# linzhiqiu/t2v_metrics

Hardware: NVIDIA B200
Metric: VQAScore (image,text) pairs/sec @ clip-flant5-xxl, 512px (higher is better)
Workload: dtype bf16

## Files before the change

t2v_metrics_b200/csrc/attention_sm100.cuh:

```cuda
#pragma once
#include "ptx.cuh"
#include "gemm_sm100.cuh"

namespace vqa {

template <typename Kernel, typename... Args>
inline cudaError_t launch_pdl(Kernel kernel, dim3 grid, dim3 block, size_t smem, cudaStream_t stream, Args... args) {
    cudaLaunchConfig_t cfg = {};
    cfg.gridDim = grid;
    cfg.blockDim = block;
    cfg.dynamicSmemBytes = smem;
    cfg.stream = stream;
    cudaLaunchAttribute attrs[1];
    attrs[0].id = cudaLaunchAttributeProgrammaticStreamSerialization;
    attrs[0].val.programmaticStreamSerializationAllowed = 1;
    cfg.attrs = attrs;
    cfg.numAttrs = pdl_enabled() ? 1 : 0;
    return cudaLaunchKernelEx(&cfg, kernel, args...);
}


constexpr int AT_BQ = 128, AT_BK = 128, AT_D = 64;
constexpr int AT_TILE_BYTES = 128 * 64 * 2;
constexpr int AT_TMEM_COLS = 256;
// ... 326 lines not shown
#pragma unroll
            for (int i = 1; i < 6; ++i) bmax_near = fmaxf(bmax_near, sRed[i]);
        }
        const uint64_t cc = pack2(p.scale_log2e, p.scale_log2e);
        const uint32_t bl2 = pack_bf16x2(b_left, b_left), br2 = pack_bf16x2(b_right, b_right);
        auto chunk_max = [](const uint32_t (&v)[32], float& m0, float& m1, float& m2, float& m3) {
#pragma unroll
            for (int i = 0; i < 32; i += 8) {
                m0 = fmax3(m0, __uint_as_float(v[i]), __uint_as_float(v[i + 1]));
                m1 = fmax3(m1, __uint_as_float(v[i + 2]), __uint_as_float(v[i + 3]));
                m2 = fmax3(m2, __uint_as_float(v[i + 4]), __uint_as_float(v[i + 5]));
                m3 = fmax3(m3, __uint_as_float(v[i + 6]), __uint_as_float(v[i + 7]));
            }
        };
        int g = 0;
        for (int qi = 0; qi < nq; ++qi) {
            const int q0 = qi * AT_BQ;
            const int qrow = q0 + row;
            __nv_bfloat16* orow = p.o + (row_base + qrow) * p.ldo + h * AT_D;
            if (q0 + (int)quad * 32 >= len) {
                for (int j = 0; j < nkt; ++j, ++g) {
                    mbar_wait(s_full, (uint32_t)g & 1u);
                    __syncwarp();
                    if (lane == 0) mbar_arrive(s_empty);
                    if (g > 0) mbar_wait(p_full, (uint32_t)(g - 1) & 1u);
                    __syncwarp();
                    if (lane == 0) mbar_arrive(p_full);
                }
                mbar_wait(o_done, (uint32_t)(g - 1) & 1u);
                __syncwarp();
                if (lane == 0) mbar_arrive(o_free);
                if (qrow < p.S) {
#pragma unroll
                    for (int c = 0; c < 8; ++c) *reinterpret_cast<uint4*>(orow + c * 8) = make_uint4(0, 0, 0, 0);
                }
                continue;
            }
            float m_run = 0.f, l_run = 0.f, corr_pend = 1.f;
            bool pend = false;
            for (int j = 0; j < nkt; ++j, ++g) {
                const int k0 = j * AT_BK;
                const int nch = min(4, (len - k0 + 31) >> 5);
                const int dt = j - qi;
                const bool near = HAS_BIAS && (dt <= p.near_tiles) && (dt >= -p.near_tiles);
                const float bias_ub = near ? bmax_near : (dt < 0 ? b_left : b_right);
                const uint32_t s_addr = tmem_S + lane_off;
                mbar_wait(s_full, (uint32_t)g & 1u);
                tcgen05_fence_after();
                if (j == 0) {
                    float a0 = -INFINITY, a1 = -INFINITY, a2 = -INFINITY, a3 = -INFINITY;
#pragma unroll 1
                    for (int c = 0; c < nch; ++c) {
                        uint32_t v[32];
                        tmem_ld_32x32b_x32(s_addr + c * 32, v);
                        tmem_ld_wait();
                        if (k0 + c * 32 + 32 > len) {
#pragma unroll
                            for (int i = 0; i < 32; ++i)
                                if (k0 + c * 32 + i >= len) v[i] = 0xff800000u;
                        }
                        chunk_max(v, a0, a1, a2, a3);
                    }
                    const float raw = fmaxf(fmaxf(a0, a1), fmaxf(a2, a3));
                    m_run = ROUND ? (raw + bias_ub) * p.scale_log2e : fmaf(raw, p.scale_log2e, bias_ub);
                } else {
                    mbar_wait(o_done, (uint32_t)(g - 1) & 1u);
                    tcgen05_fence_after();
                    if (pend) {
#pragma unroll 1
                        for (int c = 0; c < 4; ++c) {
                            uint32_t ov[16];
                            tmem_ld_32x32b_x16(tmem_O + lane_off + c * 16, ov);
                            tmem_ld_wait();
#pragma unroll
                            for (int i = 0; i < 16; ++i) ov[i] = __float_as_uint(__uint_as_float(ov[i]) * corr_pend);
                            tmem_st_32x32b_x16(tmem_O + lane_off + c * 16, ov);
                        }
                        l_run *= corr_pend;
                        pend = false;
                    }
                }
                const float a_add = near ? -m_run : (ROUND ? -m_run : bias_ub - m_run);
                const uint64_t addc = pack2(a_add, a_add);
                const uint32_t bq = near ? smem_u32(sBiasQ) + (uint32_t)(dt * 128 - row + Wn) * BQ_ENTRY : 0u;
                const uint32_t bfar = dt < 0 ? bl2 : br2;
                uint64_t acc0 = 0ull, acc1 = 0ull;
                float t0 = -INFINITY, t1 = -INFINITY, t2 = -INFINITY, t3 = -INFINITY;
                uint32_t bufA[32], bufB[32];
                auto process = [&](uint32_t (&v)[32], int c) {
                    if (c == nch - 1) {
                        tcgen05_fence_before();
                        __syncwarp();
                        if (lane == 0) mbar_arrive(s_empty);
                    }
                    if (k0 + c * 32 + 32 > len) {
#pragma unroll
                        for (int i = 0; i < 32; ++i)
                            if (k0 + c * 32 + i >= len) v[i] = 0xff800000u;
                    }
                    chunk_max(v, t0, t1, t2, t3);
                    uint32_t pk[16];
                    if (near) softmax_chunk<true, POLY, ROUND>(v, pk, bq + c * 32 * BQ_ENTRY, cc, addc, 0u, false, acc0, acc1);
                    else      softmax_chunk<false, POLY, ROUND>(v, pk, 0u, cc, addc, bfar, HAS_BIAS, acc0, acc1);
                    tmem_st_32x32b_x16(tmem_P + lane_off + c * 16, pk);
                };
                tmem_ld_32x32b_x32(s_addr, bufA);
#pragma unroll 1
                for (int c = 0; c < nch; c += 2) {
                    tmem_ld_wait();
                    if (c + 1 < nch) tmem_ld_32x32b_x32(s_addr + (c + 1) * 32, bufB);
                    process(bufA, c);
                    if (c + 1 < nch) {
                        tmem_ld_wait();
                        if (c + 2 < nch) tmem_ld_32x32b_x32(s_addr + (c + 2) * 32, bufA);
                        process(bufB, c + 1);
                    }
                }
                if (nch < 4) {
                    uint32_t z[16];
#pragma unroll
                    for (int i = 0; i < 16; ++i) z[i] = 0u;
#pragma unroll 1
                    for (int c = nch; c < 4; ++c) tmem_st_32x32b_x16(tmem_P + lane_off + c * 16, z);
                }
                {
                    float a0, a1, a2, a3;
                    unpack2(acc0, a0, a1);
                    unpack2(acc1, a2, a3);
                    l_run += (a0 + a1) + (a2 + a3);
                }
                tmem_st_wait();
                tcgen05_fence_before();
                __syncwarp();
                if (lane == 0) mbar_arrive(p_full);
                const float raw = fmaxf(fmaxf(t0, t1), fmaxf(t2, t3));
                const float bound = ROUND ? (raw + bias_ub) * p.scale_log2e : fmaf(raw, p.scale_log2e, bias_ub);
                if (__any_sync(0xffffffffu, bound > m_run + 8.f)) {
                    const float m_new = fmaxf(m_run, bound);
                    corr_pend = fast_exp2(m_run - m_new);
                    m_run = m_new;
                    pend = true;
                }
            }
            mbar_wait(o_done, (uint32_t)(g - 1) & 1u);
            tcgen05_fence_after();
            const float inv = (qrow < len) ? 1.f / l_run : 0.f;
#pragma unroll
            for (int c = 0; c < 2; ++c) {
                uint32_t ov[32];
                tmem_ld_32x32b_x32(tmem_O + lane_off + c * 32, ov);
                tmem_ld_wait();
                if (c == 1) {
                    tcgen05_fence_before();
                    __syncwarp();
                    if (lane == 0) mbar_arrive(o_free);
                }
                if (qrow < p.S) {
#pragma unroll
                    for (int gq = 0; gq < 4; ++gq) {
                        uint32_t w[4];
#pragma unroll
                        for (int e = 0; e < 4; ++e)
                            w[e] = pack_bf16x2(__uint_as_float(ov[gq * 8 + 2 * e]) * inv, __uint_as_float(ov[gq * 8 + 2 * e + 1]) * inv);
                        *reinterpret_cast<uint4*>(orow + c * 32 + gq * 8) = make_uint4(w[0], w[1], w[2], w[3]);
                    }
                }
            }
        }
        tcgen05_fence_before();
    }

    __syncthreads();
    tcgen05_fence_after();
    if (warp == 1) tmem_dealloc<1>(tmem_base, AT_TMEM_COLS);
}

template <bool HAS_BIAS, bool ROUND>
__global__ void __launch_bounds__(320, 2)
attn_tc_d64_split_kernel(const __grid_constant__ CUtensorMap tmap_qkv, const AttnTc2Params p) {
    pdl_launch_dependents();
    pdl_wait();
    constexpr int POLY = 0;
    const int h = blockIdx.y, b = blockIdx.z;
    const int len = p.seq_lens ? min(p.seq_lens[b], p.S) : p.S;
    const uint32_t warp = threadIdx.x >> 5, lane = threadIdx.x & 31u;
    const size_t row_base = (size_t)b * p.S;
    const int nq_all = (len + AT_BQ - 1) / AT_BQ;
    const int nkt = (len + AT_BK - 1) / AT_BK;
    const int q_first = blockIdx.x * p.q_per_cta;
    const int nq = max(0, min(p.q_per_cta, nq_all - q_first));

    if (blockIdx.x == 0) {
        for (int i = threadIdx.x; i < (p.S - nq_all * AT_BQ) * 8; i += blockDim.x) {
            const int r = nq_all * AT_BQ + (i >> 3), c = i & 7;
            *reinterpret_cast<uint4*>(p.o + (row_base + r) * p.ldo + h * AT_D + c * 8) = make_uint4(0, 0, 0, 0);
        }
    }
    if (nq == 0) return;

    extern __shared__ uint8_t at_smem_raw[];
    uint8_t* smem = reinterpret_cast<uint8_t*>((reinterpret_cast<uintptr_t>(at_smem_raw) + 1023) & ~uintptr_t(1023));
    uint8_t* sQ = smem;
    uint8_t* sK = smem + 2 * AT_TILE_BYTES;
    uint8_t* sV = smem + 4 * AT_TILE_BYTES;
    uint8_t* sBiasQ = smem + 6 * AT_TILE_BYTES;
    constexpr uint32_t BQ_ENTRY = ROUND ? 8u : 16u;
    const int Wn = 128 * p.near_tiles + 127;
    const int nQ = HAS_BIAS ? 2 * Wn + 1 : 0;
    float* sRed = reinterpret_cast<float*>(smem + 6 * AT_TILE_BYTES + (((size_t)nQ * BQ_ENTRY + 15) & ~size_t(15)));
    float* sXch = sRed + 16;
    uint64_t* bars = reinterpret_cast<uint64_t*>(sXch + 512);
    uint64_t* q_full = bars;
    uint64_t* q_empty = bars + 2;
    uint64_t* kv_full = bars + 4;
    uint64_t* kv_empty = bars + 6;
    uint64_t* s_full = bars + 8;
    uint64_t* s_empty = bars + 9;
    uint64_t* p_full = bars + 10;
    uint64_t* o_done = bars + 11;
    uint64_t* o_free = bars + 12;
    uint64_t* xbar = bars + 13;
    uint32_t* tmem_ptr_smem = reinterpret_cast<uint32_t*>(bars + 29);

    if (warp == 0 && lane == 0) {
        tma_prefetch_desc(&tmap_qkv);
#pragma unroll
        for (int i = 0; i < 2; ++i) {
            mbar_init(&q_full[i], 1); mbar_init(&q_empty[i], 1);
            mbar_init(&kv_full[i], 1); mbar_init(&kv_empty[i], 1);
        }
        mbar_init(s_full, 1);
        mbar_init(s_empty, 8);
        mbar_init(p_full, 8);
        mbar_init(o_done, 1);
        mbar_init(o_free, 8);
#pragma unroll
        for (int i = 0; i < 16; ++i) mbar_init(&xbar[i], 1);
        fence_barrier_init();
        mbar_arrive_expect_tx(&q_full[0], AT_TILE_BYTES);
        tma_load_2d(sQ, &tmap_qkv, &q_full[0], p.q_col0 + h * AT_D, (int)(row_base + q_first * AT_BQ));
        mbar_arrive_expect_tx(&kv_full[0], 2 * AT_TILE_BYTES);
        tma_load_2d(sK, &tmap_qkv, &kv_full[0], p.k_col0 + h * AT_D, (int)row_base);
        tma_load_2d(sV, &tmap_qkv, &kv_full[0], p.v_col0 + h * AT_D, (int)row_base);
    }
    if (warp == 1) {
        tmem_alloc<1>(tmem_ptr_smem, AT_TMEM_COLS);
        tmem_relinquish<1>();
    }
    const float LOG2E = 1.4426950408889634f;
    const float BSC = ROUND ? 1.0f : LOG2E;
    float b_left = 0.f, b_right = 0.f;
    if (HAS_BIAS) {
        const int width = 2 * p.S - 1;
        const float* src = p.bias_table + (size_t)h * width;
        b_left = __ldg(src) * BSC;
        b_right = __ldg(src + width - 1) * BSC;
        float lmax = -INFINITY;
        for (int x = threadIdx.x; x < nQ; x += blockDim.x) {
            float v[4];
#pragma unroll
            for (int k = 0; k < 4; ++k) {
                const int idx = min(max(x + k - Wn + (p.S - 1), 0), width - 1);
                v[k] = __ldg(src + idx) * BSC;
            }
            if constexpr (ROUND) reinterpret_cast<uint2*>(sBiasQ)[x] = make_uint2(pack_bf16x2(v[0], v[1]), pack_bf16x2(v[2], v[3]));
            else                 reinterpret_cast<float4*>(sBiasQ)[x] = make_float4(v[0], v[1], v[2], v[3]);
            lmax = fmaxf(lmax, v[0]);
        }
#pragma unroll
        for (int o = 16; o > 0; o >>= 1) lmax = fmaxf(lmax, __shfl_xor_sync(0xffffffffu, lmax, o));
        if (lane == 0) sRed[warp] = lmax;
    }
    tcgen05_fence_before();
    __syncthreads();
    tcgen05_fence_after();
    const uint32_t tmem_base = *tmem_ptr_smem;
    const uint32_t tmem_S = tmem_base, tmem_O = tmem_base + 128, tmem_P = tmem_base + 192;
    const int total_tiles = nq * nkt;

    if (warp == 0) {
        if (lane == 0) {
            for (int qi = 0; qi < nq; ++qi) {
                const int qb = qi & 1;
                if (qi > 0) {
                    mbar_wait(&q_empty[qb], (((uint32_t)qi >> 1) & 1u) ^ 1u);
                    mbar_arrive_expect_tx(&q_full[qb], AT_TILE_BYTES);
                    tma_load_2d(sQ + qb * AT_TILE_BYTES, &tmap_qkv, &q_full[qb], p.q_col0 + h * AT_D, (int)(row_base + (q_first + qi) * AT_BQ));
                }
                for (int j = 0; j < nkt; ++j) {
                    const int g = qi * nkt + j;
                    if (g == 0) continue;
                    const int st = g & 1;
                    mbar_wait(&kv_empty[st], (((uint32_t)g >> 1) & 1u) ^ 1u);
                    mbar_arrive_expect_tx(&kv_full[st], 2 * AT_TILE_BYTES);
                    tma_load_2d(sK + st * AT_TILE_BYTES, &tmap_qkv, &kv_full[st], p.k_col0 + h * AT_D, (int)(row_base + j * AT_BK));
                    tma_load_2d(sV + st * AT_TILE_BYTES, &tmap_qkv, &kv_full[st], p.v_col0 + h * AT_D, (int)(row_base + j * AT_BK));
                }
            }
        }
    } else if (warp == 1) {
        if (lane == 0) {
            constexpr uint32_t idesc_s = make_idesc_bf16_f32(128, 128);
            constexpr uint32_t idesc_o = make_idesc_bf16_f32(128, 64) | (1u << 16);
            auto issue_pv = [&](int g) {
                const int j = g % nkt, qi = g / nkt;
                mbar_wait(p_full, (uint32_t)g & 1u);
                if (j == 0 && qi > 0) mbar_wait(o_free, (uint32_t)(qi - 1) & 1u);
                tcgen05_fence_after();
                const uint64_t vdesc = make_mnmajor_sw128_desc(smem_u32(sV + (g & 1) * AT_TILE_BYTES), AT_TILE_BYTES);
#pragma unroll
                for (int ks = 0; ks < AT_BK / 16; ++ks)
                    umma_f16_ts(tmem_O, tmem_P + ks * 8, vdesc + (uint64_t)(ks * (16 * 128 / 16)), idesc_o,
                                (j > 0 || ks > 0) ? 1u : 0u);
                umma_commit<1>(&kv_empty[g & 1]);
                umma_commit<1>(o_done);
            };
            for (int qi = 0; qi < nq; ++qi) {
                const int qb = qi & 1;
                mbar_wait(&q_full[qb], ((uint32_t)qi >> 1) & 1u);
                const uint64_t qdesc = make_kmajor_sw128_desc(smem_u32(sQ + qb * AT_TILE_BYTES));
                for (int j = 0; j < nkt; ++j) {
                    const int g = qi * nkt + j;
                    const int st = g & 1;
                    mbar_wait(&kv_full[st], ((uint32_t)g >> 1) & 1u);
                    mbar_wait(s_empty, ((uint32_t)g & 1u) ^ 1u);
                    tcgen05_fence_after();
                    const uint64_t kdesc = make_kmajor_sw128_desc(smem_u32(sK + st * AT_TILE_BYTES));
#pragma unroll
                    for (int k = 0; k < AT_D / 16; ++k)
                        umma_f16<1>(tmem_S, qdesc + 2 * k, kdesc + 2 * k, idesc_s, k > 0 ? 1u : 0u);
                    umma_commit<1>(s_full);
                    if (j == nkt - 1) umma_commit<1>(&q_empty[qb]);
                    if (g > 0) issue_pv(g - 1);
                }
            }
            issue_pv(total_tiles - 1);
        }
    } else {
        const uint32_t quad = warp & 3u;
        const uint32_t half = (warp - 2u) >> 2;
        const int row = quad * 32 + lane;
        const uint32_t lane_off = (quad * 32u) << 16;
        uint32_t xk = 0;
        auto post = [&](float v) {
            sXch[(xk & 1u) * 256 + half * 128 + row] = v;
            __syncwarp();
            if (lane == 0) mbar_arrive(&xbar[(quad * 2 + half) * 2 + (xk & 1u)]);
        };
        auto collect = [&]() -> float {
            mbar_wait(&xbar[(quad * 2 + (half ^ 1u)) * 2 + (xk & 1u)], (xk >> 1) & 1u);
            const float other = sXch[(xk & 1u) * 256 + (half ^ 1u) * 128 + row];
            ++xk;
            return other;
        };
        float bmax_near = 0.f;
        if (HAS_BIAS) {
            bmax_near = sRed[0];
#pragma unroll
            for (int i = 1; i < 10; ++i) bmax_near = fmaxf(bmax_near, sRed[i]);
        }
        const uint64_t cc = pack2(p.scale_log2e, p.scale_log2e);
        const uint32_t bl2 = pack_bf16x2(b_left, b_left), br2 = pack_bf16x2(b_right, b_right);
        auto chunk_max = [](const uint32_t (&v)[32], float& m0, float& m1, float& m2, float& m3) {
#pragma unroll
            for (int i = 0; i < 32; i += 8) {
                m0 = fmax3(m0, __uint_as_float(v[i]), __uint_as_float(v[i + 1]));
                m1 = fmax3(m1, __uint_as_float(v[i + 2]), __uint_as_float(v[i + 3]));
                m2 = fmax3(m2, __uint_as_float(v[i + 4]), __uint_as_float(v[i + 5]));
                m3 = fmax3(m3, __uint_as_float(v[i + 6]), __uint_as_float(v[i + 7]));
            }
        };
        int g = 0;
        for (int qi = 0; qi < nq; ++qi) {
            const int q0 = (q_first + qi) * AT_BQ;
            const int qrow = q0 + row;
            __nv_bfloat16* orow = p.o + (row_base + qrow) * p.ldo + h * AT_D + half * 32;
            if (q0 + (int)quad * 32 >= len) {
                for (int j = 0; j < nkt; ++j, ++g) {
                    mbar_wait(s_full, (uint32_t)g & 1u);
                    __syncwarp();
                    if (lane == 0) mbar_arrive(s_empty);
                    if (g > 0) mbar_wait(p_full, (uint32_t)(g - 1) & 1u);
                    __syncwarp();
                    if (lane == 0) mbar_arrive(p_full);
                }
                mbar_wait(o_done, (uint32_t)(g - 1) & 1u);
                __syncwarp();
                if (lane == 0) mbar_arrive(o_free);
                if (qrow < p.S) {
#pragma unroll
                    for (int c = 0; c < 4; ++c) *reinterpret_cast<uint4*>(orow + c * 8) = make_uint4(0, 0, 0, 0);
                }
                continue;
            }
            float m_run = 0.f, l_run = 0.f;
            float bound_prev = 0.f;
            for (int j = 0; j < nkt; ++j, ++g) {
                const int k0 = j * AT_BK;
                const int nch = min(4, (len - k0 + 31) >> 5);
                const int c_lo = 2 * (int)half;
                const int n_mine = max(0, min(nch - c_lo, 2));
                const int dt = j - (q_first + qi);
                const bool near = HAS_BIAS && (dt <= p.near_tiles) && (dt >= -p.near_tiles);
                const float bias_ub = near ? bmax_near : (dt < 0 ? b_left : b_right);
                const uint32_t s_addr = tmem_S + lane_off + c_lo * 32;
                mbar_wait(s_full, (uint32_t)g & 1u);
                tcgen05_fence_after();
                uint32_t buf[32];
                auto mask = [&](uint32_t (&v)[32], int c) {
                    if (k0 + c * 32 + 32 > len) {
#pragma unroll
                        for (int i = 0; i < 32; ++i)
                            if (k0 + c * 32 + i >= len) v[i] = 0xff800000u;
                    }
                };
                bool p_free = (j == 0);
                if (j == 0) {
                    float a0 = -INFINITY, a1 = -INFINITY, a2 = -INFINITY, a3 = -INFINITY;
#pragma unroll 1
                    for (int c = 0; c < n_mine; ++c) {
                        tmem_ld_32x32b_x32(s_addr + c * 32, buf);
                        tmem_ld_wait();
                        mask(buf, c_lo + c);
                        chunk_max(buf, a0, a1, a2, a3);
                    }
                    const float raw_half = fmaxf(fmaxf(a0, a1), fmaxf(a2, a3));
                    const float bound_half = ROUND ? (raw_half + bias_ub) * p.scale_log2e : fmaf(raw_half, p.scale_log2e, bias_ub);
                    post(bound_half);
                    m_run = fmaxf(bound_half, collect());
                } else {
                    const float bound = fmaxf(bound_prev, collect());
                    if (__any_sync(0xffffffffu, bound > m_run + 8.f)) {
                        const float m_new = fmaxf(m_run, bound);
                        const float corr = fast_exp2(m_run - m_new);
                        m_run = m_new;
                        l_run *= corr;
                        mbar_wait(o_done, (uint32_t)(g - 1) & 1u);
                        tcgen05_fence_after();
                        p_free = true;
#pragma unroll 1
                        for (int c = 0; c < 2; ++c) {
                            uint32_t ov[16];
                            tmem_ld_32x32b_x16(tmem_O + lane_off + half * 32 + c * 16, ov);
                            tmem_ld_wait();
#pragma unroll
                            for (int i = 0; i < 16; ++i) ov[i] = __float_as_uint(__uint_as_float(ov[i]) * corr);
                            tmem_st_32x32b_x16(tmem_O + lane_off + half * 32 + c * 16, ov);
                        }
                    }
                }
                const float a_add = near ? -m_run : (ROUND ? -m_run : bias_ub - m_run);
                const uint64_t addc = pack2(a_add, a_add);
                const uint32_t bq = near ? smem_u32(sBiasQ) + (uint32_t)(dt * 128 - row + Wn) * BQ_ENTRY : 0u;
                const uint32_t bfar = dt < 0 ? bl2 : br2;
                uint64_t acc0 = 0ull, acc1 = 0ull;
                float t0 = -INFINITY, t1 = -INFINITY, t2 = -INFINITY, t3 = -INFINITY;
                if (n_mine == 0) {
                    __syncwarp();
                    if (lane == 0) mbar_arrive(s_empty);
                }
#pragma unroll 1
                for (int c = 0; c < 2; ++c) {
                    uint32_t pk[16];
                    if (c < n_mine) {
                        tmem_ld_32x32b_x32(s_addr + c * 32, buf);
                        tmem_ld_wait();
                        if (c == n_mine - 1) {
                            tcgen05_fence_before();
                            __syncwarp();
                            if (lane == 0) mbar_arrive(s_empty);
                        }
                        mask(buf, c_lo + c);
                        chunk_max(buf, t0, t1, t2, t3);
                        if (near) softmax_chunk<true, POLY, ROUND>(buf, pk, bq + (c_lo + c) * 32 * BQ_ENTRY, cc, addc, 0u, false, acc0, acc1);
                        else      softmax_chunk<false, POLY, ROUND>(buf, pk, 0u, cc, addc, bfar, HAS_BIAS, acc0, acc1);
                    } else {
#pragma unroll
                        for (int i = 0; i < 16; ++i) pk[i] = 0u;
                    }
                    if (!p_free) {
                        mbar_wait(o_done, (uint32_t)(g - 1) & 1u);
                        tcgen05_fence_after();
                        p_free = true;
                    }
                    tmem_st_32x32b_x16(tmem_P + lane_off + (c_lo + c) * 16, pk);
                }
                {
                    float a0, a1, a2, a3;
                    unpack2(acc0, a0, a1);
                    unpack2(acc1, a2, a3);
                    l_run += (a0 + a1) + (a2 + a3);
                }
                tmem_st_wait();
                tcgen05_fence_before();
                __syncwarp();
                if (lane == 0) mbar_arrive(p_full);
                if (j + 1 < nkt) {
                    const float raw_half = fmaxf(fmaxf(t0, t1), fmaxf(t2, t3));
                    bound_prev = ROUND ? (raw_half + bias_ub) * p.scale_log2e : fmaf(raw_half, p.scale_log2e, bias_ub);
                    post(bound_prev);
                }
            }
            post(l_run);
            const float l_row = l_run + collect();
            mbar_wait(o_done, (uint32_t)(g - 1) & 1u);
            tcgen05_fence_after();
            const float inv = (qrow < len) ? 1.f / l_row : 0.f;
            {
                uint32_t ov[32];
                tmem_ld_32x32b_x32(tmem_O + lane_off + half * 32, ov);
                tmem_ld_wait();
                tcgen05_fence_before();
                __syncwarp();
                if (lane == 0) mbar_arrive(o_free);
                if (qrow < p.S) {
#pragma unroll
                    for (int gq = 0; gq < 4; ++gq) {
                        uint32_t w[4];
#pragma unroll
                        for (int e = 0; e < 4; ++e)
                            w[e] = pack_bf16x2(__uint_as_float(ov[gq * 8 + 2 * e]) * inv, __uint_as_float(ov[gq * 8 + 2 * e + 1]) * inv);
                        *reinterpret_cast<uint4*>(orow + gq * 8) = make_uint4(w[0], w[1], w[2], w[3]);
                    }
                }
            }
        }
        tcgen05_fence_before();
    }

    __syncthreads();
    tcgen05_fence_after();
    if (warp == 1) tmem_dealloc<1>(tmem_base, AT_TMEM_COLS);
}

template <bool HAS_BIAS, bool ROUND>
inline cudaError_t launch_attn_stream_t(const CUtensorMap& tm, const AttnTc2Params& p, int B, size_t smem, cudaStream_t stream) {
    auto kernel = attn_tc_d64_stream_kernel<HAS_BIAS, ROUND>;
    static std::atomic<size_t> max_set[64];
    int dev = 0;
    cudaError_t e = cudaGetDevice(&dev);
    if (e != cudaSuccess) return e;
    if (smem > max_set[dev & 63].load(std::memory_order_acquire)) {
        e = cudaFuncSetAttribute(kernel, cudaFuncAttributeMaxDynamicSharedMemorySize, (int)smem);
        if (e != cudaSuccess) return e;
        max_set[dev & 63].store(smem, std::memory_order_release);
    }
    return launch_pdl(kernel, dim3(1, p.H, B), dim3(192), smem, stream, tm, p);
}

template <bool HAS_BIAS, bool ROUND>
inline cudaError_t launch_attn_split_t(const CUtensorMap& tm, const AttnTc2Params& p, int B, size_t smem, cudaStream_t stream, int q_ctas) {
    auto kernel = attn_tc_d64_split_kernel<HAS_BIAS, ROUND>;
    static std::atomic<size_t> max_set[64];
    int dev = 0;
    cudaError_t e = cudaGetDevice(&dev);
    if (e != cudaSuccess) return e;
    if (smem > max_set[dev & 63].load(std::memory_order_acquire)) {
        e = cudaFuncSetAttribute(kernel, cudaFuncAttributeMaxDynamicSharedMemorySize, (int)smem);
        if (e != cudaSuccess) return e;
        max_set[dev & 63].store(smem, std::memory_order_release);
    }
    return launch_pdl(kernel, dim3((unsigned)q_ctas, p.H, B), dim3(320), smem, stream, tm, p);
}

inline cudaError_t launch_attn_tc(const __nv_bfloat16* qkv, int ld, int q_col0, int k_col0, int v_col0, __nv_bfloat16* o, int ldo,
                                  int B, int S, int H, const int* seq_lens, const float* bias_table, float scale, int bias_const_from,
                                  bool round_scores, cudaStream_t stream_) {
    CUtensorMap tm;
    if (!tmap_bf16_2d_cached(&tm, qkv, (uint64_t)B * S, (uint64_t)ld, (uint64_t)ld, 128)) return cudaErrorInvalidValue;
    static const int variant = [] { const char* v = getenv("VQA_ATTN_VARIANT"); return (v && v[0]) ? atoi(v) : -1; }();
    if (variant == 30 || variant == 40) round_scores = false;
    if (variant == 31 || variant == 41) round_scores = true;
    const int stage = variant >= 40 ? 2 : (variant >= 30 ? 1 : ATTN_STAGE_DEFAULT);
    AttnTc2Params p;
    p.o = o; p.ldo = ldo; p.seq_lens = seq_lens; p.bias_table = bias_table; p.S = S; p.H = H;
    p.q_col0 = q_col0; p.k_col0 = k_col0; p.v_col0 = v_col0;
    p.scale_log2e = scale * 1.4426950408889634f;
    p.scale = scale;
    const int n_tiles = (S + 127) / 128;
    int near = n_tiles;
    if (bias_table && bias_const_from > 0 && bias_const_from < S) near = min(n_tiles, (bias_const_from - 1 + 127) / 128);
    p.near_tiles = bias_table ? near : 0;
    const size_t smem = attn_tc2_smem_bytes(p.near_tiles, bias_table != nullptr, round_scores);
    p.q_per_cta = n_tiles;
    if (stage == 2) {
        const size_t smem4 = smem + 2048 + 64 + 128;
        int q_ctas = 1;
        if (B * H < 296 && n_tiles > 1) {
            q_ctas = min(n_tiles, (296 + B * H - 1) / (B * H));
            p.q_per_cta = (n_tiles + q_ctas - 1) / q_ctas;
            q_ctas = (n_tiles + p.q_per_cta - 1) / p.q_per_cta;
        }
        if (bias_table) return round_scores ? launch_attn_split_t<true, true>(tm, p, B, smem4, stream_, q_ctas) : launch_attn_split_t<true, false>(tm, p, B, smem4, stream_, q_ctas);
        return round_scores ? launch_attn_split_t<false, true>(tm, p, B, smem4, stream_, q_ctas) : launch_attn_split_t<false, false>(tm, p, B, smem4, stream_, q_ctas);
    }
    if (bias_table) return round_scores ? launch_attn_stream_t<true, true>(tm, p, B, smem, stream_) : launch_attn_stream_t<true, false>(tm, p, B, smem, stream_);
    return round_scores ? launch_attn_stream_t<false, true>(tm, p, B, smem, stream_) : launch_attn_stream_t<false, false>(tm, p, B, smem, stream_);
}

struct AttnTc128Params {
    __nv_bfloat16* o;
    int ldo;
    const int* cu_seqlens;
    const int* seq_lens;
    int S;
    int q_col0, k_col0, v_col0;
    int kv_group;
    float scale_log2e;
    int o_head_stride, d_out;
    int pair, n_seq;
    const int* kv_prefix;
};

constexpr int A8_TILE = 128 * 128 * 2;
constexpr int A8_BLOCK = 128 * 64 * 2;
constexpr int A8_TMEM_COLS = 512;
inline size_t attn_tc128_smem_bytes() { return 1024 + 5 * A8_TILE + 128; }

template <bool CAUSAL, int POLY>
__global__ void __launch_bounds__(192, 1)
attn_tc_d128_kernel(const __grid_constant__ CUtensorMap tmap_qkv, const AttnTc128Params p) {
    pdl_launch_dependents();
    pdl_wait();
    const int qt = blockIdx.x, h = blockIdx.y, b = blockIdx.z;
    const int kvh = h / p.kv_group;
    const uint32_t warp = threadIdx.x >> 5, lane = threadIdx.x & 31u;
    int row_base, len, write_rows, mid = 0;
    if (p.cu_seqlens && p.pair) {
        row_base = p.cu_seqlens[2 * b];
        mid = p.cu_seqlens[2 * b + 1] - row_base;
        len = p.cu_seqlens[min(2 * b + 2, p.n_seq)] - row_base;
        write_rows = len;
    } else if (p.cu_seqlens) {
        row_base = p.cu_seqlens[b];
        len = p.cu_seqlens[b + 1] - row_base;
        write_rows = len;
    } else {
        row_base = b * p.S;
        len = p.seq_lens ? min(p.seq_lens[b], p.S) : p.S;
// ... 258 lines not shown
```

t2v_metrics_b200/csrc/ptx.cuh:

```cuda
#pragma once
#include <cstdlib>
#include <cuda_runtime.h>
#include <cuda_bf16.h>
#include <stdint.h>

namespace vqa {

__device__ __forceinline__ uint32_t smem_u32(const void* p) {
    return static_cast<uint32_t>(__cvta_generic_to_shared(p));
}
__device__ __forceinline__ uint32_t lane_id() { return threadIdx.x & 31u; }

__device__ __forceinline__ bool elect_one() {
    uint32_t pred = 0;
    asm volatile(
        "{\n\t"
        ".reg .pred P;\n\t"
        "elect.sync _|P, 0xffffffff;\n\t"
        "selp.b32 %0, 1, 0, P;\n\t"
        "}\n"
        : "=r"(pred));
    return pred != 0;
}

__device__ __forceinline__ uint32_t cluster_ctarank() {
    uint32_t r;
    asm volatile("mov.u32 %0, %%cluster_ctarank;" : "=r"(r));
    return r;
}
__device__ __forceinline__ void cluster_sync_all() {
    asm volatile("barrier.cluster.arrive.release.aligned;\n\tbarrier.cluster.wait.acquire.aligned;" ::: "memory");
}

__device__ __forceinline__ void mbar_init(uint64_t* bar, uint32_t count) {
    asm volatile("mbarrier.init.shared::cta.b64 [%0], %1;" ::"r"(smem_u32(bar)), "r"(count) : "memory");
}
__device__ __forceinline__ void fence_barrier_init() {
    asm volatile("fence.mbarrier_init.release.cluster;" ::: "memory");
}
__device__ __forceinline__ void fence_proxy_async_smem() {
    asm volatile("fence.proxy.async.shared::cta;" ::: "memory");
}
__device__ __forceinline__ void mbar_wait(uint64_t* bar, uint32_t parity) {
    asm volatile(
        "{\n\t"
        ".reg .pred P1;\n\t"
        "WAIT_LOOP:\n\t"
        "mbarrier.try_wait.parity.shared::cta.b64 P1, [%0], %1, %2;\n\t"
        "@P1 bra WAIT_DONE;\n\t"
        "bra WAIT_LOOP;\n\t"
        "WAIT_DONE:\n\t"
        "}\n" ::"r"(smem_u32(bar)),
        "r"(parity), "r"(0x989680u)
        : "memory");
}
__device__ __forceinline__ void pdl_launch_dependents() { asm volatile("griddepcontrol.launch_dependents;" ::: "memory"); }
__device__ __forceinline__ void pdl_wait() { asm volatile("griddepcontrol.wait;" ::: "memory"); }
inline bool pdl_enabled() {
    static const bool on = [] { const char* v = getenv("VQA_PDL"); return v && v[0] == '1'; }();
    return on;
}

__device__ __forceinline__ void mbar_wait_spin(uint64_t* bar, uint32_t parity) {
    asm volatile(
        "{\n\t"
        ".reg .pred P1;\n\t"
        "WAIT_LOOP:\n\t"
        "mbarrier.try_wait.parity.shared::cta.b64 P1, [%0], %1;\n\t"
        "@P1 bra WAIT_DONE;\n\t"
        "bra WAIT_LOOP;\n\t"
        "WAIT_DONE:\n\t"
        "}\n" ::"r"(smem_u32(bar)),
        "r"(parity)
        : "memory");
}
__device__ __forceinline__ void mbar_arrive(uint64_t* bar) {
    asm volatile("mbarrier.arrive.shared::cta.b64 _, [%0];" ::"r"(smem_u32(bar)) : "memory");
}
__device__ __forceinline__ void mbar_arrive_expect_tx(uint64_t* bar, uint32_t bytes) {
    asm volatile("mbarrier.arrive.expect_tx.shared::cta.b64 _, [%0], %1;" ::"r"(smem_u32(bar)), "r"(bytes)
                 : "memory");
}
__device__ __forceinline__ void mbar_arrive_cluster(uint64_t* bar, uint32_t cta) {
    asm volatile(
        "{\n\t"
        ".reg .b32 remAddr32;\n\t"
        "mapa.shared::cluster.u32 remAddr32, %0, %1;\n\t"
        "mbarrier.arrive.shared::cluster.b64 _, [remAddr32];\n\t"
        "}\n" ::"r"(smem_u32(bar)),
        "r"(cta)
        : "memory");
}

__device__ __forceinline__ void tma_prefetch_desc(const void* desc) {
    asm volatile("prefetch.tensormap [%0];" ::"l"(reinterpret_cast<uint64_t>(desc)) : "memory");
}
constexpr uint64_t L2_EVICT_NORMAL = 0x1000000000000000ull;
constexpr uint64_t L2_EVICT_FIRST = 0x12F0000000000000ull;
constexpr uint64_t L2_EVICT_LAST = 0x14F0000000000000ull;

__device__ __forceinline__ void tma_load_2d_hint(void* smem_dst, const void* desc, uint64_t* bar, int32_t c0, int32_t c1,
                                                 uint64_t policy) {
    asm volatile(
        "cp.async.bulk.tensor.2d.shared::cluster.global.mbarrier::complete_tx::bytes.L2::cache_hint"
        " [%0], [%1, {%3, %4}], [%2], %5;" ::"r"(smem_u32(smem_dst)),
        "l"(reinterpret_cast<uint64_t>(desc)), "r"(smem_u32(bar)), "r"(c0), "r"(c1), "l"(policy)
        : "memory");
}
__device__ __forceinline__ void tma_load_2d_2sm_hint(void* smem_dst, const void* desc, uint64_t* bar, int32_t c0, int32_t c1,
                                                     uint64_t policy) {
    uint32_t bar_addr = smem_u32(bar) & 0xFEFFFFFFu;
    asm volatile(
        "cp.async.bulk.tensor.2d.cta_group::2.shared::cluster.global.mbarrier::complete_tx::bytes.L2::cache_hint"
        " [%0], [%1, {%3, %4}], [%2], %5;" ::"r"(smem_u32(smem_dst)),
        "l"(reinterpret_cast<uint64_t>(desc)), "r"(bar_addr), "r"(c0), "r"(c1), "l"(policy)
        : "memory");
}

__device__ __forceinline__ void tma_load_2d(void* smem_dst, const void* desc, uint64_t* bar, int32_t c0,
                                            int32_t c1) {
    asm volatile(
        "cp.async.bulk.tensor.2d.shared::cluster.global.mbarrier::complete_tx::bytes"
        " [%0], [%1, {%3, %4}], [%2];" ::"r"(smem_u32(smem_dst)),
        "l"(reinterpret_cast<uint64_t>(desc)), "r"(smem_u32(bar)), "r"(c0), "r"(c1)
        : "memory");
}
__device__ __forceinline__ void tma_load_2d_2sm(void* smem_dst, const void* desc, uint64_t* bar, int32_t c0,
                                                int32_t c1) {
    uint32_t bar_addr = smem_u32(bar) & 0xFEFFFFFFu;
    asm volatile(
        "cp.async.bulk.tensor.2d.cta_group::2.shared::cluster.global.mbarrier::complete_tx::bytes"
        " [%0], [%1, {%3, %4}], [%2];" ::"r"(smem_u32(smem_dst)),
        "l"(reinterpret_cast<uint64_t>(desc)), "r"(bar_addr), "r"(c0), "r"(c1)
        : "memory");
}

template <int CG>
__device__ __forceinline__ void tmem_alloc(uint32_t* smem_dst, uint32_t ncols) {
    if constexpr (CG == 1)
        asm volatile("tcgen05.alloc.cta_group::1.sync.aligned.shared::cta.b32 [%0], %1;" ::"r"(smem_u32(smem_dst)),
                     "r"(ncols)
                     : "memory");
    else
        asm volatile("tcgen05.alloc.cta_group::2.sync.aligned.shared::cta.b32 [%0], %1;" ::"r"(smem_u32(smem_dst)),
                     "r"(ncols)
                     : "memory");
}
template <int CG>
__device__ __forceinline__ void tmem_relinquish() {
    if constexpr (CG == 1)
        asm volatile("tcgen05.relinquish_alloc_permit.cta_group::1.sync.aligned;" ::: "memory");
    else
        asm volatile("tcgen05.relinquish_alloc_permit.cta_group::2.sync.aligned;" ::: "memory");
}
template <int CG>
__device__ __forceinline__ void tmem_dealloc(uint32_t taddr, uint32_t ncols) {
    if constexpr (CG == 1)
        asm volatile("tcgen05.dealloc.cta_group::1.sync.aligned.b32 %0, %1;" ::"r"(taddr), "r"(ncols) : "memory");
    else
        asm volatile("tcgen05.dealloc.cta_group::2.sync.aligned.b32 %0, %1;" ::"r"(taddr), "r"(ncols) : "memory");
}
__device__ __forceinline__ void tcgen05_fence_before() {
    asm volatile("tcgen05.fence::before_thread_sync;" ::: "memory");
}
__device__ __forceinline__ void tcgen05_fence_after() {
    asm volatile("tcgen05.fence::after_thread_sync;" ::: "memory");
}

template <int CG>
__device__ __forceinline__ void umma_f16(uint32_t tmem_d, uint64_t adesc, uint64_t bdesc, uint32_t idesc,
                                         uint32_t accumulate) {
    if constexpr (CG == 1)
        asm volatile(
            "{\n\t"
            ".reg .pred p;\n\t"
            "setp.ne.b32 p, %4, 0;\n\t"
            "tcgen05.mma.cta_group::1.kind::f16 [%0], %1, %2, %3, p;\n\t"
            "}\n" ::"r"(tmem_d),
            "l"(adesc), "l"(bdesc), "r"(idesc), "r"(accumulate)
            : "memory");
    else
        asm volatile(
            "{\n\t"
            ".reg .pred p;\n\t"
            "setp.ne.b32 p, %4, 0;\n\t"
            "tcgen05.mma.cta_group::2.kind::f16 [%0], %1, %2, %3, p;\n\t"
            "}\n" ::"r"(tmem_d),
            "l"(adesc), "l"(bdesc), "r"(idesc), "r"(accumulate)
            : "memory");
}
template <int CG>
__device__ __forceinline__ void umma_commit(uint64_t* bar) {
    if constexpr (CG == 1)
        asm volatile("tcgen05.commit.cta_group::1.mbarrier::arrive::one.shared::cluster.b64 [%0];" ::"r"(
                         smem_u32(bar))
                     : "memory");
    else
        asm volatile(
            "tcgen05.commit.cta_group::2.mbarrier::arrive::one.shared::cluster.multicast::cluster.b64 [%0], %1;" ::
                "r"(smem_u32(bar)),
            "h"(static_cast<uint16_t>(3))
            : "memory");
}

__device__ __forceinline__ void tmem_ld_32x32b_x32(uint32_t taddr, uint32_t (&r)[32]) {
    asm volatile(
        "tcgen05.ld.sync.aligned.32x32b.x32.b32 "
        "{%0, %1, %2, %3, %4, %5, %6, %7, %8, %9, %10, %11, %12, %13, %14, %15, "
        "%16, %17, %18, %19, %20, %21, %22, %23, %24, %25, %26, %27, %28, %29, %30, %31}, [%32];"
        : "=r"(r[0]), "=r"(r[1]), "=r"(r[2]), "=r"(r[3]), "=r"(r[4]), "=r"(r[5]), "=r"(r[6]), "=r"(r[7]),
          "=r"(r[8]), "=r"(r[9]), "=r"(r[10]), "=r"(r[11]), "=r"(r[12]), "=r"(r[13]), "=r"(r[14]), "=r"(r[15]),
          "=r"(r[16]), "=r"(r[17]), "=r"(r[18]), "=r"(r[19]), "=r"(r[20]), "=r"(r[21]), "=r"(r[22]),
          "=r"(r[23]), "=r"(r[24]), "=r"(r[25]), "=r"(r[26]), "=r"(r[27]), "=r"(r[28]), "=r"(r[29]),
          "=r"(r[30]), "=r"(r[31])
        : "r"(taddr)
        : "memory");
}
__device__ __forceinline__ void tmem_ld_wait() { asm volatile("tcgen05.wait::ld.sync.aligned;" ::: "memory"); }

__device__ __forceinline__ uint64_t make_kmajor_sw128_desc(uint32_t smem_addr) {
    uint64_t d = 0;
    d |= static_cast<uint64_t>((smem_addr >> 4) & 0x3FFFu);
    d |= static_cast<uint64_t>(1) << 16;
    d |= static_cast<uint64_t>(1024 >> 4) << 32;
    d |= static_cast<uint64_t>(1) << 46;
    d |= static_cast<uint64_t>(2) << 61;
    return d;
}
__host__ __device__ constexpr uint32_t make_idesc_bf16_f32(uint32_t umma_m, uint32_t umma_n) {
    return (1u << 4)
           | (1u << 7)
           | (1u << 10)
           | ((umma_n >> 3) << 17)
           | ((umma_m >> 4) << 24);
}

__device__ __forceinline__ float bf16_round(float x) { return __bfloat162float(__float2bfloat16_rn(x)); }
__device__ __forceinline__ uint32_t pack_bf16x2(float lo, float hi) {
    __nv_bfloat162 v = __floats2bfloat162_rn(lo, hi);
    return *reinterpret_cast<uint32_t*>(&v);
}
__device__ __forceinline__ float2 unpack_bf16x2(uint32_t u) {
    __nv_bfloat162 v = *reinterpret_cast<__nv_bfloat162*>(&u);
    return __bfloat1622float2(v);
}

}
```

Baseline: 166.0.

## Poll barriers in attention MMA warp and issue PV MMAs opportunistically

The attention MMA-issuing thread no longer blocks in turn on the Q, KV and S-empty barriers. It polls them with non-blocking mbarrier test_wait and, while waiting, issues any pending P·V MMA whose P tile and O buffer are ready. This aims to let QK^T and PV MMAs interleave dynamically instead of in a fixed one-behind order, keeping the tensor core busier. It adds polling overhead with nanosleep backoff, and the reordering could raise TMEM hazards if barrier parity reasoning is off.

After: 165.6 (median of 6 runs). About the same (-0.2%).

```diff
diff --git a/t2v_metrics_b200/csrc/attention_sm100.cuh b/t2v_metrics_b200/csrc/attention_sm100.cuh
--- a/t2v_metrics_b200/csrc/attention_sm100.cuh
+++ b/t2v_metrics_b200/csrc/attention_sm100.cuh
@@ -652,6 +652,10 @@
         if (lane == 0) {
             constexpr uint32_t idesc_s = make_idesc_bf16_f32(128, 128);
             constexpr uint32_t idesc_o = make_idesc_bf16_f32(128, 64) | (1u << 16);
+            auto pv_ready = [&](int g) {
+                const int j = g % nkt, qi = g / nkt;
+                return mbar_test(p_full, (uint32_t)g & 1u) && (j > 0 || qi == 0 || mbar_test(o_free, (uint32_t)(qi - 1) & 1u));
+            };
             auto issue_pv = [&](int g) {
                 const int j = g % nkt, qi = g / nkt;
                 mbar_wait(p_full, (uint32_t)g & 1u);
@@ -665,15 +669,22 @@
                 umma_commit<1>(&kv_empty[g & 1]);
                 umma_commit<1>(o_done);
             };
+            int next_pv = 0;
             for (int qi = 0; qi < nq; ++qi) {
                 const int qb = qi & 1;
-                mbar_wait(&q_full[qb], ((uint32_t)qi >> 1) & 1u);
                 const uint64_t qdesc = make_kmajor_sw128_desc(smem_u32(sQ + qb * AT_TILE_BYTES));
                 for (int j = 0; j < nkt; ++j) {
                     const int g = qi * nkt + j;
                     const int st = g & 1;
-                    mbar_wait(&kv_full[st], ((uint32_t)g >> 1) & 1u);
-                    mbar_wait(s_empty, ((uint32_t)g & 1u) ^ 1u);
+                    bool q_ok = j > 0, kv_ok = false, s_ok = false;
+                    for (;;) {
+                        q_ok = q_ok || mbar_test(&q_full[qb], ((uint32_t)qi >> 1) & 1u);
+                        kv_ok = kv_ok || mbar_test(&kv_full[st], ((uint32_t)g >> 1) & 1u);
+                        s_ok = s_ok || mbar_test(s_empty, ((uint32_t)g & 1u) ^ 1u);
+                        if (q_ok && kv_ok && s_ok) break;
+                        if (next_pv < g && pv_ready(next_pv)) issue_pv(next_pv++);
+                        else __nanosleep(32);
+                    }
                     tcgen05_fence_after();
                     const uint64_t kdesc = make_kmajor_sw128_desc(smem_u32(sK + st * AT_TILE_BYTES));
 #pragma unroll
@@ -681,10 +692,10 @@
                         umma_f16<1>(tmem_S, qdesc + 2 * k, kdesc + 2 * k, idesc_s, k > 0 ? 1u : 0u);
                     umma_commit<1>(s_full);
                     if (j == nkt - 1) umma_commit<1>(&q_empty[qb]);
-                    if (g > 0) issue_pv(g - 1);
-                }
-            }
-            issue_pv(total_tiles - 1);
+                    if (next_pv < g && pv_ready(next_pv)) issue_pv(next_pv++);
+                }
+            }
+            while (next_pv < total_tiles) issue_pv(next_pv++);
         }
     } else {
         const uint32_t quad = warp & 3u;
diff --git a/t2v_metrics_b200/csrc/ptx.cuh b/t2v_metrics_b200/csrc/ptx.cuh
--- a/t2v_metrics_b200/csrc/ptx.cuh
+++ b/t2v_metrics_b200/csrc/ptx.cuh
@@ -53,6 +53,19 @@
         "}\n" ::"r"(smem_u32(bar)),
         "r"(parity), "r"(0x989680u)
         : "memory");
+}
+__device__ __forceinline__ bool mbar_test(uint64_t* bar, uint32_t parity) {
+    uint32_t ok;
+    asm volatile(
+        "{\n\t"
+        ".reg .pred P1;\n\t"
+        "mbarrier.test_wait.parity.shared::cta.b64 P1, [%1], %2;\n\t"
+        "selp.b32 %0, 1, 0, P1;\n\t"
+        "}\n"
+        : "=r"(ok)
+        : "r"(smem_u32(bar)), "r"(parity)
+        : "memory");
+    return ok != 0;
 }
 __device__ __forceinline__ void pdl_launch_dependents() { asm volatile("griddepcontrol.launch_dependents;" ::: "memory"); }
 __device__ __forceinline__ void pdl_wait() { asm volatile("griddepcontrol.wait;" ::: "memory"); }
```
